# isislovecruft/aeonflux

Measured on AMD Instinct MI355X. Metric: credential presentations verified/sec, higher is better.
Workload: dtype int64

## Files before the change

aeonflux_amd/csrc/engine.cpp:

```cpp
#include "engine.hpp"
#include <stdio.h>
#include <string.h>
#include <algorithm>
#include <map>
#include <tuple>
#include <new>
#include <system_error>
#include <stdexcept>

namespace afx {

static thread_local std::string g_error;
void set_error(const std::string& s) { g_error = s; }
int exception_rc() noexcept {
  try {
    throw;
  } catch (const std::bad_alloc&) {
    try { set_error("out of host memory"); } catch (...) {}
    return AFX_E_NO_MEMORY;
  } catch (const std::system_error& e) {
    try { set_error(std::string("system: ") + e.what()); } catch (...) {}
    return AFX_E_NO_MEMORY;
  } catch (const std::exception& e) {
    try { set_error(std::string("internal: ") + e.what()); } catch (...) {}
// ... 18 lines not shown
    if (e != hipSuccess) { set_error(std::string("hipFree: ") + hipGetErrorString(e)); return AFX_E_HIP; }
  }
  const size_t want = (n + (size_t(1) << 20) - 1) & ~((size_t(1) << 20) - 1);
  hipError_t e = hipMalloc(&p, want);
  if (e != hipSuccess) { p = nullptr; g_alloc_failed = true; set_error("hipMalloc(" + std::to_string(want) + "): " + hipGetErrorString(e)); return AFX_E_HIP; }
  cap = want;
  return AFX_OK;
}
void DevBuf::release(bool wipe) {
  if (!p) return;
  if (wipe) (void)hipMemset(p, 0, cap);
  (void)hipFree(p);
  p = nullptr; cap = 0;
}

static void secure_zero(void* p, size_t n) {
  if (!n) return;
  memset(p, 0, n);
  __asm__ __volatile__("" : : "r"(p) : "memory");
}
Assembler::~Assembler() { secure_zero(blob_.data(), blob_.size()); }
static uint8_t* provisional_base(int range, int variant) { return (uint8_t*)(uintptr_t)(0x4000000000000000ull + ((uint64_t)(1 + range + 4 * variant) << 44)); }
Assembler::Assembler(afx_ctx* c, uint32_t cnt, int variant) : ctx(c), count(cnt) {
  blob_.reserve(1 << 16);
  blob_base_ = provisional_base(0, variant);
  ws_base_ = provisional_base(1, variant);
  blob_alloc(sizeof(afx_pass), 16);
  bad_ = (uint32_t*)ws_alloc(sizeof(uint32_t) * (size_t)count);
  Launch l;
  l.kind = L_FILL_BAD;
  l.njobs = 1;
  l.jobs_off = blob_alloc(sizeof(afx_fill_job), 16);
  launches.push_back(l);
}
uint8_t* Assembler::ws_alloc(size_t bytes) {
  const size_t off = (ws_off_ + 255) & ~size_t(255);
  ws_off_ = off + bytes;
  return ws_base_ + off;
}
int32_t* Assembler::new_var() { return (int32_t*)ws_alloc(sizeof(int32_t) * AFX_VAR_DWORDS * (size_t)count); }
uint8_t* Assembler::new_enc() { return ws_alloc(32 * (size_t)count); }
uint8_t* Assembler::new_wide() { return ws_alloc(64 * (size_t)count); }
uint8_t* Assembler::new_rows(size_t rows) { return ws_alloc(32 * rows * (size_t)count); }
uint64_t* Assembler::new_state() { return (uint64_t*)ws_alloc(sizeof(uint64_t) * 25 * (size_t)count); }
size_t Assembler::blob_alloc(size_t bytes, size_t align) {
  const size_t off = (blob_.size() + align - 1) & ~(align - 1);
  blob_.resize(off + bytes);
  return off;
}
template <class T> static void put_job(uint8_t* dst, const T& j) { memcpy(dst, &j, sizeof j); }
template <> void put_job(uint8_t* dst, const afx_decode_job& j) {
  afx_decode_job z; memset(&z, 0, sizeof z);
  z.enc = j.enc; z.out = j.out; z.reject_identity = j.reject_identity; z.elligator = j.elligator;
  memcpy(dst, &z, sizeof z);
}
template <> void put_job(uint8_t* dst, const afx_pointop_job& j) {
  afx_pointop_job z; memset(&z, 0, sizeof z);
  z.a = j.a; z.b = j.b; z.b_const = j.b_const; z.sa = j.sa; z.sb = j.sb; z.out = j.out; z.out_enc = j.out_enc; z.reject_identity = j.reject_identity;
  memcpy(dst, &z, sizeof z);
}
template <> void put_job(uint8_t* dst, const afx_scalarop_job& j) {
  afx_scalarop_job z; memset(&z, 0, sizeof z);
  z.a = j.a; z.a_stride = j.a_stride; z.b = j.b; z.b_stride = j.b_stride; z.c = j.c; z.c_stride = j.c_stride; z.negate = j.negate; z.out = j.out;
  memcpy(dst, &z, sizeof z);
}
template <LaunchKind K, class T>
void Assembler::add_jobs(const std::vector<T>& jobs) {
  static_assert(job_of_kind<T>(K), "not the job struct of this launch kind");
  if (jobs.empty()) return;
  Launch l;
  l.kind = K;
  l.njobs = (uint32_t)jobs.size();
  l.jobs_off = blob_alloc(sizeof(T) * jobs.size(), 16);
  for (size_t i = 0; i < jobs.size(); i++) put_job(blob_.data() + l.jobs_off + sizeof(T) * i, jobs[i]);
  launches.push_back(l);
}
void Assembler::decode(const std::vector<afx_decode_job>& jobs) {
  stats.decodings += jobs.size();
  stats.field_mul += AFX_DECODE_MUL * jobs.size();
  stats.field_sq += AFX_DECODE_SQ * jobs.size();
  stats.chain_mul += AFX_CHAIN_SQRT_MUL * jobs.size();
  stats.chain_sq += AFX_CHAIN_SQRT_SQ * jobs.size();
  if (!pending_maps_.empty()) {
    std::vector<afx_decode_job> all(pending_maps_);
    all.insert(all.end(), jobs.begin(), jobs.end());
    pending_maps_.clear();
    add_jobs(all);
    launches.back().odd = 1;
    flush_maps();
    return;
  }
  add_jobs(jobs);
}
void Assembler::flush_maps() {
  if (!pending_maps_.empty()) {
    std::vector<afx_decode_job> maps;
    maps.swap(pending_maps_);
    add_jobs(maps);
    launches.back().odd = 1;
  }
  if (!pending_map_sums_.empty()) {
    std::vector<afx_pointop_job> sums;
    sums.swap(pending_map_sums_);
    pointop(sums);
  }
}
void Assembler::sccheck(const std::vector<afx_sccheck_job>& jobs) { add_jobs(jobs); }
void Assembler::pointop(const std::vector<afx_pointop_job>& jobs) {
  flush_maps();
  for (const afx_pointop_job& j : jobs) {
    stats.var_additions += j.sb != 0;
    stats.encodings += j.out_enc != nullptr;
    stats.field_mul += (j.sb != 0 ? 9 : 0) + (j.out_enc ? AFX_ENCODE_MUL : 0);
    stats.field_sq += j.out_enc ? AFX_ENCODE_SQ : 0;
    stats.chain_mul += j.out_enc ? AFX_CHAIN_SQRT_MUL : 0;
    stats.chain_sq += j.out_enc ? AFX_CHAIN_SQRT_SQ : 0;
  }
  if (small() && (uint64_t)ctx->row_waves(count) * jobs.size() <= 2ull * 4 * ctx->n_cu) {
    std::vector<afx_pointop_job> moved(jobs);
    for (afx_pointop_job& j : moved) {
      if (!j.out_enc || j.reject_identity == 2) continue;
      if (!j.out) j.out = new_var();
      afx_compress_job cj = { j.out, j.out_enc, j.reject_identity, AFX_COMPRESS_PLAIN };
      pending_cjobs_.push_back(cj);
      j.out_enc = nullptr; j.reject_identity = 0;
    }
    add_jobs(moved);
    return;
  }
  add_jobs(jobs);
}
void Assembler::negenc(const std::vector<afx_negenc_job>& jobs) {
  flush_maps();
  if (jobs.empty()) return;
  stats.encodings += jobs.size();
  stats.field_mul += 11 + (2 * 3 + 2 + 17) * jobs.size();
  stats.field_sq += 254 + 3 * jobs.size();
  stats.chain_mul += AFX_CHAIN_INVERT_MUL; stats.chain_sq += AFX_CHAIN_INVERT_SQ;
  add_jobs(jobs);
  add_walk_rows(launches.back(), 0);
}
void Assembler::add_walk_rows(Launch& l, uint32_t per_row) {
  if (per_row == 0 || per_row > l.njobs) per_row = l.njobs;
  std::vector<afx_walk_row> rows;
  for (uint32_t first = 0; first < l.njobs; first += per_row) {
// ... 1329 lines not shown
```

aeonflux_amd/csrc/kernels.hip:

```cpp
#include <hip/hip_runtime.h>
#include "ge.cuh"
#include "keccak.cuh"
#include "plan.h"
#include "sc.cuh"
#include "sha512.cuh"

AFX_DEV void enc_load(uint32_t w[8], const uint8_t* arr, uint32_t item) {
  const uint4* p = reinterpret_cast<const uint4*>(arr + 32ull * item);
  const uint4 a = p[0], b = p[1];
  w[0] = a.x; w[1] = a.y; w[2] = a.z; w[3] = a.w; w[4] = b.x; w[5] = b.y; w[6] = b.z; w[7] = b.w;
}
AFX_DEV void enc_store(uint8_t* arr, uint32_t item, const uint32_t w[8]) {
  uint4* p = reinterpret_cast<uint4*>(arr + 32ull * item);
  p[0] = make_uint4(w[0], w[1], w[2], w[3]);
  p[1] = make_uint4(w[4], w[5], w[6], w[7]);
}
AFX_DEV sc sc_load_item(const uint8_t* arr, uint32_t stride, uint32_t item) {
  uint32_t w[8];
  enc_load(w, arr, stride ? item : 0);
  sc r;
#pragma unroll
  for (int i = 0; i < 8; i++) r.v[i] = w[i];
  return r;
}
// ... 115 lines not shown
    Q = ge_double(Q);
    if ((c >> bit) & 1u) Q = ge_p1p1_to_p3(ge_add_cached(Q, cB, false));
  }
#pragma unroll 1
  for (int k = 0; k < 4; k++) Q = ge_double(Q);
  int32_t* tab = postab + (size_t)(gj / windows) * windows * window_dwords + (size_t)(gj % windows) * window_dwords;
  const uint32_t first = c * AFX_POS_CHUNK, n = min((uint32_t)AFX_POS_CHUNK, entries - first);
  fe X[AFX_POS_CHUNK], Y[AFX_POS_CHUNK], Z[AFX_POS_CHUNK], pre[AFX_POS_CHUNK];
  fe prod = fe_one();
#pragma unroll 1
  for (uint32_t k = 0; k < n; k++) {
    X[k] = Q.X; Y[k] = Q.Y; Z[k] = Q.Z; pre[k] = prod;
    prod = fe_mul(prod, Q.Z);
    if (k + 1 < n) Q = ge_p1p1_to_p3(ge_add_cached(Q, cB, false));
  }
  fe inv = fe_invert(prod);
#pragma unroll 1
  for (int k = (int)n - 1; k >= 0; k--) {
    const fe zinv = fe_mul(inv, pre[k]);
    inv = fe_mul(inv, Z[k]);
    const ge_niels q = ge_niels_from_affine(fe_mul(X[k], zinv), fe_mul(Y[k], zinv));
    int32_t* e = tab + (size_t)(first + k) * AFX_NIELS_DWORDS;
#pragma unroll
    for (int l = 0; l < AFX_FE_LIMBS; l++) { e[l] = q.ypx.v[l]; e[9 + l] = q.ymx.v[l]; e[18 + l] = q.xyd.v[l]; }
    e[27] = 0;
  }
}

template <class T>
AFX_DEV const T* row_job(const T* __restrict__ jobs, const afx_row* __restrict__ rows) {
  if (rows) return reinterpret_cast<const T*>(reinterpret_cast<const uint8_t*>(jobs) + rows[blockIdx.y].job_off);
  return jobs + blockIdx.y;
}
AFX_DEV uint32_t row_pass_index(const afx_row* __restrict__ rows) { return rows ? rows[blockIdx.y].pass : 0u; }
template <class T> struct lane_row { T job; uint32_t count; uint32_t* bad; uint32_t item; };
template <class T>
AFX_DEV lane_row<T> lane_row_of(const T* __restrict__ jobs, const afx_row* __restrict__ rows, const afx_pass* __restrict__ passes) {
  const afx_pass pass = passes[row_pass_index(rows)];
  return { *row_job(jobs, rows), pass.count, pass.bad, blockIdx.x * blockDim.x + threadIdx.x };
}
AFX_DEV bool wave_past_end(uint32_t count) {
  return blockIdx.x * blockDim.x + ((uint32_t)__builtin_amdgcn_readfirstlane((int)threadIdx.x) & ~63u) >= count;
}
AFX_DEV uint32_t shadowing_item(uint32_t count) { return min(blockIdx.x * blockDim.x + threadIdx.x, count - 1); }
struct quad_seat { uint32_t lane, role, item; };
AFX_DEV quad_seat quad_seat_of(uint32_t count) {
  const uint32_t lane = threadIdx.x & 63u;
  return { lane, (uint32_t)__builtin_amdgcn_readfirstlane((int)(threadIdx.x >> 6)), min(blockIdx.x * 64u + lane, count - 1) };
}

AFX_DEV void decode_item(const afx_decode_job& job, uint32_t* bad, uint32_t count, uint32_t item) {
  uint32_t w[8];
  enc_load(w, job.enc, item);
  ge_p3 P;
  const bool ok = ristretto_decode(P, w);
  uint32_t flags = ok ? 0u : AFX_BAD_DECODE;
  if (job.reject_identity && is_identity_encoding(w)) flags |= AFX_BAD_IDENTITY;
  if (flags) atomicOr(&bad[item], flags);
  if (job.out) var_store(job.out, count, item, ok ? P : ge_identity());
}
__global__ void __launch_bounds__(AFX_BLOCK, 2) k_decode(const afx_decode_job* __restrict__ jobs, const afx_row* __restrict__ rows, const afx_pass* __restrict__ passes) {
  const auto [job, count, bad, item] = lane_row_of(jobs, rows, passes);
  if (item >= count) return;
  decode_item(job, bad, count, item);
}

__global__ void __launch_bounds__(AFX_BLOCK) k_decode_mixed(const afx_decode_job* __restrict__ jobs, const afx_row* __restrict__ rows, const afx_pass* __restrict__ passes) {
  const auto [job, count, bad, item] = lane_row_of(jobs, rows, passes);
  if (item >= count) return;
  if (job.elligator) {
    uint32_t w[8];
    enc_load(w, job.enc, 2 * item + (job.elligator - 1));
    var_store(job.out, count, item, ristretto_elligator(fe_frombytes(w)));
    return;
  }
  decode_item(job, bad, count, item);
}

__global__ void __launch_bounds__(AFX_BLOCK) k_sccheck(const afx_sccheck_job* __restrict__ jobs, const afx_row* __restrict__ rows, const afx_pass* __restrict__ passes) {
  const auto [job, count, bad, item] = lane_row_of(jobs, rows, passes);
  if (item >= count) return;
  const sc s = sc_load_item(job.sc, 32, item);
  if (!sc_is_canonical(s)) atomicOr(&bad[item], AFX_BAD_SCALAR);
}

__global__ void __launch_bounds__(AFX_BLOCK, 2) k_pointop(const afx_pointop_job* __restrict__ jobs, const afx_row* __restrict__ rows, const afx_pass* __restrict__ passes) {
  const auto [job, count, bad, item] = lane_row_of(jobs, rows, passes);
  if (item >= count) return;
  ge_p3 A = var_load(job.a, count, item);
  if (job.sa < 0) A = ge_neg(A);
  ge_p3 R = A;
  if (job.sb != 0) {
    const ge_p3 B = job.b ? var_load(job.b, count, item) : p3_load_uniform(job.b_const);
    R = ge_addsub(A, B, job.sb < 0);
  } else {
    R = ge_carry(R);
  }
  if (job.out) var_store(job.out, count, item, R);
  if (job.out_enc) {
    uint32_t w[8];
    ristretto_encode(w, R);
    enc_store(job.out_enc, item, w);
    if (job.reject_identity == 1 ? is_identity_encoding(w) : (job.reject_identity == 2 && !is_identity_encoding(w))) atomicOr(&bad[item], AFX_BAD_IDENTITY);
  }
}

// ... 1471 lines not shown
```

aeonflux_amd/csrc/launch_kinds.hpp:

```cpp
#pragma once
#include <stddef.h>
#include <stdint.h>
#include <string>
#include "../../include/aeonflux_gpu.h"
#include "kernels.h"
#include "plan.h"

hipError_t afxk_coef(hipStream_t s, const afx_coef_job* jobs, uint32_t njobs, const afx_row* rows, const afx_pass* passes, uint32_t max_count) __attribute__((weak));
hipError_t afxk_mask_rows(hipStream_t s, const afx_mask_job* jobs, uint32_t njobs, const afx_row* rows, const afx_pass* passes, uint32_t max_count) __attribute__((weak));
hipError_t afxk_sha512_jobs(hipStream_t s, const afx_sha512_job* jobs, uint32_t njobs, const afx_row* rows, const afx_pass* passes, uint32_t max_count) __attribute__((weak));
hipError_t afxk_encode_to_group(hipStream_t s, const afx_encode_job* jobs, uint32_t njobs, const afx_row* rows, const afx_pass* passes, uint32_t max_count) __attribute__((weak));
hipError_t afxk_encode_at(hipStream_t s, const afx_encode_at_job* jobs, uint32_t njobs, const afx_row* rows, const afx_pass* passes, uint32_t max_count) __attribute__((weak));
hipError_t afxk_sha512(hipStream_t s, const uint8_t* src, uint32_t stride, uint32_t offset, uint32_t len, uint8_t* out, uint32_t count) __attribute__((weak));
hipError_t afxk_draw(hipStream_t s, const afx_draw_job* jobs, uint32_t njobs, uint32_t max_count) __attribute__((weak));
hipError_t afxk_batch_weights(hipStream_t s, const uint8_t* seed, uint64_t index0, uint32_t label, uint32_t n_weights, uint32_t count, uint8_t* weights) __attribute__((weak));
hipError_t afxk_msg_gather(hipStream_t s, const afx_gather_job* job) __attribute__((weak));
hipError_t afxk_msg_expand(hipStream_t s, const afx_expand_job* job) __attribute__((weak));
hipError_t afxk_msg_status(hipStream_t s, const afx_msgstat_job* job) __attribute__((weak));
hipError_t afxk_sc_invert(hipStream_t s, const uint8_t* a, const uint8_t* b, uint8_t* out, uint32_t count) __attribute__((weak));
hipError_t afxk_tag_broadcast(hipStream_t s, const uint8_t* enc, uint8_t* rows, uint32_t count) __attribute__((weak));
hipError_t afxk_tag_scope_check(hipStream_t s, const uint8_t* enc, uint8_t* ok) __attribute__((weak));
hipError_t afxk_tagset_spend(hipStream_t s, const afx_tagset_table* t, const uint8_t* T, const uint8_t* status_in, uint32_t count, uint32_t* slot_of, uint8_t* seen_out)
    __attribute__((weak));
hipError_t afxk_tagset_contains(hipStream_t s, const afx_tagset_table* t, const uint8_t* T, uint32_t count, uint8_t* seen_out) __attribute__((weak));
// ... 19 lines not shown
  void fix(const T*& p) const { T* q = const_cast<T*>(p); fix(q); p = q; }
  template <class T, size_t N>
  void fix(T (&a)[N]) const { for (T& p : a) fix(p); }
};
template <class J, auto... M>
void fix_jobs(const Mover& m, uint8_t* j0, uint32_t n) {
  for (uint32_t i = 0; i < n; i++) {
    J& j = ((J*)j0)[i];
    (m.fix(j.*M), ...);
  }
}
enum OddRule { ODD_IGNORED, ODD_EQUAL, ODD_OR };

struct KindInfo {
  LaunchKind kind;
  const char* name;
  size_t job_size;
  const char* job_type;
  void (*fix)(const Mover& m, uint8_t* jobs, uint32_t njobs);
  bool walks;
  OddRule odd;
  int (*run)(const KindInfo& k, hipStream_t s, const uint8_t* jobs, uint32_t njobs, const afx_row* rows, const afx_pass* passes, uint32_t max_count);
  const char* call;
};

template <class J> constexpr const char* job_tag() { return __PRETTY_FUNCTION__; }
constexpr bool same_text(const char* a, const char* b) { while (*a && *a == *b) a++, b++; return *a == *b; }
template <class J>
using Launcher = hipError_t(hipStream_t, const J*, uint32_t, const afx_row*, const afx_pass*, uint32_t);
template <class J, Launcher<J>* F, bool OPTIONAL>
int run_common(const KindInfo& k, hipStream_t s, const uint8_t* jobs, uint32_t njobs, const afx_row* rows, const afx_pass* passes, uint32_t max_count) {
  if constexpr (OPTIONAL)
    if (!F) { set_error(std::string("no ") + k.name + " launcher in this build"); return AFX_E_NO_DEVICE; }
  const hipError_t e = F(s, (const J*)jobs, njobs, rows, passes, max_count);
  if (e != hipSuccess) { set_error(std::string(k.call) + ": " + hipGetErrorString(e)); return AFX_E_HIP; }
  return AFX_OK;
}
#define AFX_COMMON(J, F) &run_common<J, F, false>, #F "(s, (const " #J "*)jobs, nrows, rw, passes, max_count)"
#define AFX_OPTIONAL(J, F) &run_common<J, F, true>, #F "(s, (const " #J "*)jobs, nrows, rw, passes, max_count)"

template <class J, auto... M>
constexpr KindInfo kind_of(LaunchKind k, const char* name, bool walks = false, OddRule odd = ODD_IGNORED, decltype(KindInfo::run) run = nullptr, const char* call = nullptr) {
  return { k, name, sizeof(J), job_tag<J>(), &fix_jobs<J, M...>, walks, odd, run, call };
}
template <class J, auto... M>
constexpr KindInfo kind_of(LaunchKind k, const char* name, decltype(KindInfo::run) run, const char* call) { return kind_of<J, M...>(k, name, false, ODD_IGNORED, run, call); }

constexpr KindInfo msm_kind(LaunchKind k, const char* name) {
  return kind_of<afx_msm_djob, &afx_msm_djob::naf_sched, &afx_msm_djob::addend, &afx_msm_djob::out_enc, &afx_msm_djob::out_var, &afx_msm_djob::half_var>(k, name);
}

inline constexpr KindInfo KINDS[] = {
  kind_of<afx_fill_job, &afx_fill_job::p>(L_FILL_BAD, "k_fill_u32"),
  kind_of<afx_decode_job, &afx_decode_job::enc, &afx_decode_job::out>(L_DECODE, "k_decode", false, ODD_OR),
  kind_of<afx_sccheck_job, &afx_sccheck_job::sc>(L_SCCHECK, "k_sccheck", AFX_COMMON(afx_sccheck_job, afxk_sccheck)),
  kind_of<afx_pointop_job, &afx_pointop_job::a, &afx_pointop_job::b, &afx_pointop_job::b_const, &afx_pointop_job::out, &afx_pointop_job::out_enc>(
      L_POINTOP, "k_pointop", AFX_COMMON(afx_pointop_job, afxk_pointop)),
  kind_of<afx_scalarop_job, &afx_scalarop_job::a, &afx_scalarop_job::b, &afx_scalarop_job::c, &afx_scalarop_job::out>(
      L_SCALAROP, "k_scalarop", AFX_COMMON(afx_scalarop_job, afxk_scalarop)),
  msm_kind(L_MSM_WINDOW, "k_msm_window"),
  kind_of<afx_hash_program, &afx_hash_program::init_state, &afx_hash_program::load_state, &afx_hash_program::save_state, &afx_hash_program::records,
          &afx_hash_program::fields, &afx_hash_program::outs, &afx_hash_program::challenge, &afx_hash_program::trace>(L_HASH, "k_hash"),
  kind_of<afx_uniform_job, &afx_uniform_job::wide, &afx_uniform_job::out_enc, &afx_uniform_job::out_var>(
      L_FROM_UNIFORM, "k_from_uniform", AFX_COMMON(afx_uniform_job, afxk_from_uniform_jobs)),
  kind_of<afx_reduce_job, &afx_reduce_job::wide, &afx_reduce_job::out>(L_REDUCE_WIDE, "k_reduce_wide", AFX_COMMON(afx_reduce_job, afxk_reduce_wide_jobs)),
  { L_COPY, "copy", 0, nullptr, nullptr, false, ODD_IGNORED, nullptr, nullptr },
  kind_of<afx_finish_job, &afx_finish_job::bad, &afx_finish_job::status>(L_FINISH, "k_finish"),
  msm_kind(L_MSM_FIXED, "k_msm_fixed"),
  msm_kind(L_MSM_NAF, "k_msm_naf"),
  kind_of<afx_table_job, &afx_table_job::var>(L_MSM_TABLES, "k_msm_tables", false, ODD_EQUAL),
  kind_of<afx_compress_job, &afx_compress_job::var, &afx_compress_job::out_enc>(L_COMPRESS, "k_compress2x", true),
  kind_of<afx_pointsum_job, &afx_pointsum_job::parts, &afx_pointsum_job::addend, &afx_pointsum_job::out_var, &afx_pointsum_job::half_var, &afx_pointsum_job::out_enc>(
      L_POINTSUM, "k_pointsum", false, ODD_OR),
  kind_of<afx_negenc_job, &afx_negenc_job::enc, &afx_negenc_job::var, &afx_negenc_job::out_enc>(L_NEGENC, "k_negenc", true),
  kind_of<afx_table_job, &afx_table_job::var>(L_TABLE_AFFINE, "k_table_affine", true),
  kind_of<afx_powers_job, &afx_powers_job::src, &afx_powers_job::out>(L_POWERS, "k_powers", AFX_COMMON(afx_powers_job, afxk_powers)),
  kind_of<afx_coef_job, &afx_coef_job::weights, &afx_coef_job::triples, &afx_coef_job::operands, &afx_coef_job::out>(L_COEF, "k_coef", AFX_OPTIONAL(afx_coef_job, afxk_coef)),
  kind_of<afx_sha512_job, &afx_sha512_job::src, &afx_sha512_job::out, &afx_sha512_job::copy>(L_SHA512, "k_sha512", AFX_OPTIONAL(afx_sha512_job, afxk_sha512_jobs)),
  kind_of<afx_encode_job, &afx_encode_job::msgs, &afx_encode_job::M1, &afx_encode_job::counters, &afx_encode_job::zero_a, &afx_encode_job::zero_b>(
      L_ENCODE, "k_encode_to_group", AFX_OPTIONAL(afx_encode_job, afxk_encode_to_group)),
  kind_of<afx_mask_job, &afx_mask_job::p>(L_MASK, "k_mask_rows", AFX_OPTIONAL(afx_mask_job, afxk_mask_rows)),
  kind_of<afx_encode_at_job, &afx_encode_at_job::msgs, &afx_encode_at_job::counters_in, &afx_encode_at_job::M1, &afx_encode_at_job::zero_a, &afx_encode_at_job::zero_b>(
      L_ENCODE_AT, "k_encode_at", AFX_OPTIONAL(afx_encode_at_job, afxk_encode_at)),
};
#undef AFX_COMMON
#undef AFX_OPTIONAL
inline constexpr const char* TIMING_SLOT_NAMES[] = { "k_hash_coop", "k_hash_coop64", "k_sc_invert" };

constexpr bool kinds_in_enum_order() {
  for (int k = 0; k < (int)L_KINDS; k++) if (KINDS[k].kind != k) return false;
  return true;
}
static_assert(sizeof KINDS / sizeof KINDS[0] == L_KINDS && kinds_in_enum_order(), "one KINDS entry per launch kind, in the enum's order");
static_assert(sizeof TIMING_SLOT_NAMES / sizeof TIMING_SLOT_NAMES[0] == T_SLOTS - L_KINDS, "one name per timing slot past the launch kinds");
inline const KindInfo& kind_info(LaunchKind k) { return KINDS[k]; }
inline const char* timing_name(int slot) { return slot < (int)L_KINDS ? KINDS[slot].name : TIMING_SLOT_NAMES[slot - L_KINDS]; }

template <class J>
constexpr bool job_of_kind(LaunchKind k) { return KINDS[k].job_type && same_text(KINDS[k].job_type, job_tag<J>()); }
template <class J>
constexpr LaunchKind kind_of_job() {
  int found = L_KINDS, n = 0;
  for (int k = 0; k < (int)L_KINDS; k++) if (job_of_kind<J>((LaunchKind)k)) { found = k; n++; }
  return n == 1 ? (LaunchKind)found : L_KINDS;
}

}
// ... 1 lines not shown
```

aeonflux_amd/csrc/plan.h:

```cpp
#pragma once
#include <stdint.h>

#define AFX_KV_ONE_WAVE_CHAINS 0x08u
#define AFX_KV_HASH_HALF_WAVE 0x10u
#define AFX_KV_NO_POINTSUM_TREE 0x20u

#define AFX_CLOCK_SLOTS 64
#define AFX_MSM_MAX_TERMS 72
#define AFX_TABLE_ENTRIES 9
#define AFX_TABLE_STORED 8
#ifndef AFX_POS_BITS
#define AFX_POS_BITS 13
#endif
#define AFX_POS_WINDOWS ((253 + AFX_POS_BITS - 1) / AFX_POS_BITS)
#define AFX_POS_ENTRIES ((1 << (AFX_POS_BITS - 1)) + 1)
#define AFX_POS_WINDOW_DWORDS ((AFX_POS_ENTRIES * AFX_NIELS_DWORDS + 3) & ~3)
#define AFX_POS_TABLE_DWORDS (AFX_POS_WINDOWS * AFX_POS_WINDOW_DWORDS)
#define AFX_SEC_BITS 6
#define AFX_SEC_WINDOWS ((253 + AFX_SEC_BITS - 1) / AFX_SEC_BITS)
#define AFX_SEC_ENTRIES ((1 << (AFX_SEC_BITS - 1)) + 1)
#define AFX_SEC_WINDOW_DWORDS (AFX_SEC_ENTRIES * AFX_NIELS_DWORDS)
#define AFX_SEC_TABLE_DWORDS (AFX_SEC_WINDOWS * AFX_SEC_WINDOW_DWORDS)
#ifndef AFX_SECVAR_BITS
#define AFX_SECVAR_BITS 2
// ... 37 lines not shown
  uint32_t pass;
  uint32_t job_off;
} afx_row;

typedef struct {
  uint32_t job_off;
  uint32_t n_jobs;
  uint32_t pass, pad;
  int32_t* prefix_ws;
} afx_walk_row;

typedef struct { uint32_t* p; uint32_t v, n; } afx_fill_job;
typedef struct { const uint32_t* bad; uint8_t* status; uint32_t count, fail_code; } afx_finish_job;
typedef struct { uint8_t* p; } afx_mask_job;
typedef struct { const uint8_t* wide; uint8_t* out_enc; int32_t* out_var; } afx_uniform_job;
typedef struct { const uint8_t* wide; uint8_t* out; } afx_reduce_job;
typedef struct { const uint8_t* src; uint8_t* out; uint8_t* copy; uint32_t stride, offset, len, pad; } afx_sha512_job;
typedef struct { const uint8_t* msgs; uint8_t* M1; uint32_t* counters; uint8_t* zero_a; uint8_t* zero_b; } afx_encode_job;
typedef struct { const uint8_t* msgs; const uint32_t* counters_in; uint8_t* M1; uint8_t* zero_a; uint8_t* zero_b; } afx_encode_at_job;

typedef struct { const uint8_t* blob; const uint64_t* offsets; const uint32_t* chunk_first; uint8_t* rows; uint64_t bias; uint32_t count, n_chunks; } afx_gather_job;
#define AFX_EXPAND_MAX 3
typedef struct { const uint8_t* src[AFX_EXPAND_MAX]; uint8_t* dst[AFX_EXPAND_MAX]; const uint32_t* chunk_first; uint32_t count, n_chunks, n_rows; } afx_expand_job;
typedef struct {
  const uint8_t* chunk_status[2]; uint8_t* status; const uint32_t* chunk_first;
  const uint8_t* keys[AFX_EXPAND_MAX];
  uint8_t* rows32[2]; uint8_t* rows30; uint32_t* words;
  uint32_t count, n_chunks, n_keys, fail_code, phase, pad;
} afx_msgstat_job;

typedef struct { const uint8_t* seed; uint8_t* dst; uint64_t index; uint32_t count, label; } afx_draw_job;
#define AFX_DRAW_LEN(label) (((label) == 0u || (label) == 1u || (label) == 3u || ((label) >= 65u && (label) <= 67u) || (label) == 69u || \
                              ((label) >= 71u && (label) <= 102u)) ? 64u : 32u)

#define AFX_COEF_ONE 0xffffu
typedef struct { uint16_t weight, operand, negate, pad; } afx_coef_triple;
typedef struct {
  const uint8_t* weights;
  const afx_coef_triple* triples;
  const uint8_t* const* operands;
  uint8_t* out;
  uint64_t stride;
  uint32_t n_triples, pad;
} afx_coef_job;
#define AFX_WEIGHT_BYTES 16u

typedef int32_t* afx_var_t;

typedef struct {
  const uint8_t* enc;
  afx_var_t out;
  uint32_t reject_identity;
  uint32_t elligator;
} afx_decode_job;

typedef struct {
  const uint8_t* sc;
} afx_sccheck_job;

typedef struct {
  const int32_t* a;
  const int32_t* b;
  const int32_t* b_const;
  int32_t sa, sb;
  afx_var_t out;
  uint8_t* out_enc;
  uint32_t reject_identity;
} afx_pointop_job;

typedef struct {
  const uint8_t* a; uint32_t a_stride;
  const uint8_t* b; uint32_t b_stride;
  const uint8_t* c; uint32_t c_stride;
  uint32_t negate;
  uint8_t* out;
} afx_scalarop_job;

typedef struct {
  const uint8_t* scalar;
  uint32_t scalar_stride;
  int32_t fixed_idx;
  const int32_t* var;
  uint32_t negate;
  uint32_t table_slot;
  uint32_t secret;
  uint32_t dbl;
  uint32_t win_off;
  uint32_t pad;
} afx_msm_term;

typedef struct {
  uint32_t n_terms;
  uint32_t n_var;
  uint32_t n_uni;
  int32_t top_bit;
  const uint32_t* naf_sched;
  afx_msm_term term[AFX_MSM_MAX_TERMS];
  const int32_t* addend;
  uint32_t addend_negate;
  uint8_t* out_enc;
  afx_var_t out_var;
  uint32_t reject_identity;
  uint32_t leave_half;
  int32_t chain_to;
  afx_var_t half_var;
  uint32_t digit_slot;
// ... 119 lines not shown
```

aeonflux_amd/csrc/statements.cpp:

```cpp
#include <string.h>
#include <algorithm>
#include <functional>
#include <memory>
#include <stdexcept>
#include <vector>
#include "engine.hpp"
#include <stdlib.h>
#include "doors.hpp"

using namespace afx;

static const uint8_t SC_L_BYTES[32] = { 0xed, 0xd3, 0xf5, 0x5c, 0x1a, 0x63, 0x12, 0x58, 0xd6, 0x9c, 0xf7, 0xa2, 0xde, 0xf9, 0xde, 0x14,
                                        0, 0, 0, 0, 0, 0, 0, 0, 0, 0, 0, 0, 0, 0, 0, 0x10 };
static bool host_scalar_is_canonical(const uint8_t* s) {
  for (int i = 31; i >= 0; i--) {
    if (s[i] < SC_L_BYTES[i]) return true;
    if (s[i] > SC_L_BYTES[i]) return false;
  }
  return false;
}
static size_t sizeof_system_parameters(uint32_t n) { return n < 3 ? 32 * (5 + 3 + (size_t)n + 4) + 4 : 32 * (5 + 2 * (size_t)n + 4) + 4; }
static size_t sizeof_secret_key(uint32_t n) { return 32 * (5 + (size_t)n) + 4; }


// ... 330 lines not shown
      if (k >= 2) continue;
      if ((rc = L.blob_dev[i].ensure(BLOB_CAP))) return rc;
      AFX_HIP(hipHostMalloc(&L.blob_host[i], BLOB_CAP, hipHostMallocDefault));
      L.blob_host_cap[i] = BLOB_CAP;
    }
  for (auto& L : c->lane) AFX_HIP(hipEventCreateWithFlags(&L.msm_done, hipEventDisableTiming));
  std::vector<uint8_t> flat(32 * (size_t)c->ngen);
  for (uint32_t i = 0; i < c->ngen; i++) memcpy(flat.data() + 32 * (size_t)i, c->gen_enc[i].data(), 32);
  AFX_HIP(hipMemcpyAsync(c->d_gen_enc.p, flat.data(), flat.size(), hipMemcpyHostToDevice, c->stream));
  uint8_t* d_neg = (uint8_t*)c->lane[0].staging.p;
  uint32_t* d_ok = (uint32_t*)((uint8_t*)c->lane[0].staging.p + 32 * (size_t)c->ngen);
  AFX_HIP(afxk_setup_generators(c->stream, (const uint8_t*)c->d_gen_enc.p, c->ngen, (int32_t*)c->d_gen_ext.p, d_neg, d_ok));
  if ((rc = c->lane[0].ws.ensure(sizeof(int32_t) * AFX_VAR_DWORDS * (size_t)c->ngen * AFX_POS_WINDOWS))) return rc;
  AFX_HIP(afxk_setup_postables(c->stream, (const int32_t*)c->d_gen_ext.p, c->ngen, (int32_t*)c->lane[0].ws.p, (int32_t*)c->d_pos_tables.p, 0));
  std::vector<uint8_t> neg(32 * (size_t)c->ngen);
  std::vector<uint32_t> ok(c->ngen);
  AFX_HIP(hipMemcpyAsync(neg.data(), d_neg, neg.size(), hipMemcpyDeviceToHost, c->stream));
  AFX_HIP(hipMemcpyAsync(ok.data(), d_ok, 4 * (size_t)c->ngen, hipMemcpyDeviceToHost, c->stream));
  if (c->has_key) {
    std::vector<uint8_t> kflat(32 * (size_t)(4 + n));
    for (uint32_t i = 0; i < 4 + n; i++) memcpy(kflat.data() + 32 * (size_t)i, c->host_key[i].data(), 32);
    AFX_HIP(hipMemcpyAsync(c->d_key.p, kflat.data(), kflat.size(), hipMemcpyHostToDevice, c->stream));
    AFX_HIP(hipStreamSynchronize(c->stream));
    volatile uint8_t* p = kflat.data();
    for (size_t i = 0; i < kflat.size(); i++) p[i] = 0;
  }
  uint8_t consts[2048];
  memset(consts, 0, sizeof consts);
  consts[0] = 1;
  AFX_HIP(hipMemcpyAsync(c->d_consts.p, consts, sizeof consts, hipMemcpyHostToDevice, c->stream));
  AFX_HIP(hipStreamSynchronize(c->stream));
  for (uint32_t i = 0; i < c->ngen; i++)
    if (!ok[i]) { set_error("generator / key point " + std::to_string(i) + " does not decompress"); return AFX_E_BAD_PARAMS; }
  c->gen_neg_enc.assign(c->ngen, Enc{});
  for (uint32_t i = 0; i < c->ngen; i++) memcpy(c->gen_neg_enc[i].data(), neg.data() + 32 * (size_t)i, 32);
  if ((rc = build_secret_tables(c.get()))) return rc;
  *out = c.release();
  return AFX_OK;
}

extern "C" int afx_ctx_create(afx_ctx** out, int device, const uint8_t* sysparams, size_t sysparams_len, const uint8_t* amacs_key,
                              size_t amacs_key_len, const uint8_t issuer_params[64]) try {
  if (!issuer_params) { set_error("issuer_params is required"); return AFX_E_BAD_ARGS; }
  return afx_ctx_create_impl(out, device, sysparams, sysparams_len, amacs_key, amacs_key_len, nullptr, issuer_params);
} catch (...) { return afx::exception_rc(); }

struct BatchableIn {
  const uint8_t* main = nullptr;
  const uint8_t* const* enc = nullptr;
  uint32_t n_main = 0;
  const uint8_t* weights = nullptr;
  BatchableSum sum;
};
static void add_encproof_verify(Assembler& as, JobSets& js, uint16_t index, const afx_encproof_soa& e, size_t total, size_t off, uint32_t trace_row,
                                BatchableSum* sum = nullptr, const uint8_t* commitments = nullptr) {
  afx_ctx* c = as.ctx;
  auto row = [&](const uint8_t* base, size_t k) { return base + (k * total + off) * 32; };
  if (index >= c->n) { as.fail_all = true; return; }
  if (!sum) js.sccheck.push_back({ row(e.challenge, 0) });
  for (int k = 0; k < 6; k++) js.sccheck.push_back({ row(e.responses, k) });
  int32_t *v_pk = as.new_var(), *v_E1 = as.new_var(), *v_E2 = as.new_var(), *v_Cy1 = as.new_var(), *v_Cy2 = as.new_var(),
          *v_Cy3 = as.new_var(), *v_Cy2p = as.new_var(), *v_D1 = as.new_var();
  uint8_t *e_D1 = as.new_enc(), *e_D2 = as.new_enc();
  js.decode.push_back({ row(e.pk, 0), v_pk, 1 });
  js.decode.push_back({ row(e.E1, 0), v_E1, 1 });
  js.decode.push_back({ row(e.E2, 0), v_E2, 0 });
  js.decode.push_back({ row(e.C_y_1, 0), v_Cy1, 0 });
  js.decode.push_back({ row(e.C_y_2, 0), v_Cy2, 1 });
  js.decode.push_back({ row(e.C_y_3, 0), v_Cy3, 1 });
  js.decode.push_back({ row(e.C_y_2p, 0), v_Cy2p, 1 });
  afx_pointop_job d1 = { v_Cy1, v_E2, nullptr, +1, -1, v_D1, e_D1, 1 };
  js.pointop.push_back(d1);
  if (as.small()) js.pointop.push_back({ v_E1, nullptr, nullptr, -1, 0, nullptr, e_D2, 1 });
  else js.negenc.push_back({ row(e.E1, 0), v_E1, e_D2, 1, 0 });
  auto resp = [&](int k) { ScalarVar s; s.dev = row(e.responses, k); s.stride = 32; return s; };
  SchnorrBuilder v(as, "2019/1416 anonymous credentials", "2019/1416 proof of encryption");
  const int a = v.allocate_scalar("a", resp(0));
  const int a0 = v.allocate_scalar("a0", resp(1));
  const int a1 = v.allocate_scalar("a1", resp(2));
  const int m3 = v.allocate_scalar("m3", resp(3));
  const int z = v.allocate_scalar("z", resp(4));
  const int z1 = v.allocate_scalar("z1", resp(5));
  const int pk = v.allocate_point("pk", PointVar::Var(v_pk, row(e.pk, 0)));
  const int G_a = v.allocate_point("G_a", PointVar::Const(c->id_Ga()));
  const int G_a_0 = v.allocate_point("G_a_0", PointVar::Const(c->id_Ga0()));
  const int G_a_1 = v.allocate_point("G_a_1", PointVar::Const(c->id_Ga1()));
  const int G_y_1 = v.allocate_point("G_y_1", PointVar::Const(c->id_Gy(0)));
  const int G_y_2 = v.allocate_point("G_y_2", PointVar::Const(c->id_Gy(1)));
  const int G_y_3 = v.allocate_point("G_y_3", PointVar::Const(c->id_Gy(2)));
  const int G_m_3 = v.allocate_point("G_m_3", PointVar::Const(c->id_Gm(index)));
  const int C_y_2 = v.allocate_point("C_y_2", PointVar::Var(v_Cy2, row(e.C_y_2, 0)));
  const int C_y_3 = v.allocate_point("C_y_3", PointVar::Var(v_Cy3, row(e.C_y_3, 0)));
  const int C_y_2p = v.allocate_point("C_y_2'", PointVar::Var(v_Cy2p, row(e.C_y_2p, 0)));
  const int C_y_1_minus_E2 = v.allocate_point("C_y_1-E2", PointVar::Var(v_D1, e_D1));
  const int E1 = v.allocate_point("E1", PointVar::Var(v_E1, row(e.E1, 0)));
  const int minus_E1 = v.allocate_point("-E1", PointVar::NegOf(v_E1, e_D2));
  v.constrain(pk, { { a, G_a }, { a0, G_a_0 }, { a1, G_a_1 } });
  v.constrain(C_y_1_minus_E2, { { z, G_y_1 }, { a, minus_E1 } });
  v.constrain(C_y_2p, { { a1, C_y_2 } });
  v.constrain(E1, { { a0, C_y_2 }, { m3, C_y_2p }, { z1, G_y_2 } });
  v.constrain(C_y_3, { { z, G_y_3 }, { m3, G_m_3 } });
  if (sum) {
    const uint8_t* R[5];
    for (size_t j = 0; j < 5; j++) R[j] = row(commitments, j);
    if (!v.verify_batchable(R, 5, trace_row, total, off, *sum, js.decode, js.hash)) throw std::logic_error("a proof of encryption has five constraints");
    return;
  }
  v.verify_compact(row(e.challenge, 0), trace_row, total, off, js.msm1, js.hash);
}

static void add_tagproof_verify(Assembler& as, JobSets& js, std::vector<afx_msm_job>& chains, const TagVerify& tv, const int32_t* v_Cyp, size_t total, size_t off,
                                uint32_t trace_row) {
  afx_ctx* c = as.ctx;
  const uint32_t p = tv.position;
  if (p >= c->n) { as.fail_all = true; return; }
  auto row = [&](const uint8_t* base, size_t k) { return base + (k * total + off) * 32; };
  js.sccheck.push_back({ row(tv.nonce, 0) });
  js.sccheck.push_back({ row(tv.challenge, 0) });
  for (int k = 0; k < 2; k++) js.sccheck.push_back({ row(tv.responses, k) });
  int32_t *v_T = as.new_var(), *v_H = as.new_var(), *v_Cp = as.new_var();
// ... 35 lines not shown
    if (sh.kinds[i] > AFX_ENC_SECRET_POINT) return true;
  for (uint32_t j = 0; j < hs; j++)
    if (sh.hidden_scalar_indices[j] >= c->n) return true;
  for (uint32_t e = 0; e < sh.n_enc_proofs; e++)
    if (sh.enc_indices[e] >= c->n) return true;
  uint32_t k = 0;
  for (uint32_t i = 0; i < n; i++)
    if (sh.kinds[i] != AFX_ENC_SECRET_POINT) keep[k++] = i;
  if (c->strict) {
    uint32_t e = 0;
    for (uint32_t i = 0; i < n; i++)
      if (sh.kinds[i] == AFX_ENC_SECRET_POINT) {
        if (e >= sh.n_enc_proofs || sh.enc_indices[e] != i) return true;
        e++;
      }
    if (e != sh.n_enc_proofs) return true;
  }
  for (uint32_t j = 0; j < k; j++) {
    const uint32_t p = c->strict ? keep[j] : j;
    pos[j] = p;
    hidden_slot[j] = -1;
    if (sh.kinds[p] == AFX_ENC_SECRET_POINT) continue;
    if (p >= c->g) return true;
    if (sh.kinds[p] == AFX_ENC_SECRET_SCALAR) {
      for (uint32_t h = 0; h < hs; h++)
        if (sh.hidden_scalar_indices[h] == p) { hidden_slot[j] = (int)h; break; }
      if (hidden_slot[j] < 0) return true;
    }
  }
  *k_out = k;
  return false;
}

static void build_presentation_verify(Assembler& as, const afx_shape& sh, const afx_presentation_soa& b, size_t total, size_t off,
                                      uint8_t* status_dev, BatchableIn* bi = nullptr, const TagVerify* tv = nullptr) {
  afx_ctx* c = as.ctx;
  JobSets js;
  auto row = [&](const uint8_t* base, size_t k) { return base + (k * total + off) * 32; };
  const uint32_t n = sh.n_attributes, hs = sh.n_hidden_scalars;
  uint32_t keep[AFX_MAX_ATTRIBUTES], pos[AFX_MAX_ATTRIBUTES], k = 0;
  int hidden_slot[AFX_MAX_ATTRIBUTES];
  if (presentation_shape_rejects(c, sh, keep, &k, hidden_slot, pos)) as.fail_all = true;
  if (tv && (bi || !tagged_shape_ok(c, sh, tv->position))) as.fail_all = true;
  if (as.fail_all) { emit(as, js, status_dev, AFX_ST_VERIFICATION_FAILURE); return; }

  if (!bi) js.sccheck.push_back({ row(b.challenge, 0) });
  for (uint32_t r = 0; r < sh.n_responses; r++) js.sccheck.push_back({ row(b.responses, r) });
  int32_t *v_Cx0 = as.new_var(), *v_Cx1 = as.new_var(), *v_CV = as.new_var(), *v_A = as.new_var(), *v_Z = as.new_var();
  uint8_t* e_Z = as.new_enc();
  js.decode.push_back({ row(b.C_x_0, 0), v_Cx0, 1 });
  js.decode.push_back({ row(b.C_x_1, 0), v_Cx1, 1 });
  js.decode.push_back({ row(b.C_V, 0), v_CV, 0 });
  int32_t* v_Cy[AFX_MAX_ATTRIBUTES];
  std::vector<afx_msm_term> zterms;
  zterms.push_back(mk_term(c->key_x0(), 0, v_Cx0, -1, true));
  zterms.push_back(mk_term(c->key_x1(), 0, v_Cx1, -1, true));
  for (uint32_t i = 0; i < n; i++) {
    v_Cy[i] = as.new_var();
    js.decode.push_back({ row(b.C_y, i), v_Cy[i], sh.kinds[i] != AFX_ENC_SECRET_POINT ? 1u : 0u });
    const int32_t* X = v_Cy[i];
    if (sh.kinds[i] == AFX_ENC_PUBLIC_SCALAR) {
      js.sccheck.push_back({ row(b.attr_values, i) });
      uint8_t* ym = as.new_enc();
      afx_scalarop_job so;
      memset(&so, 0, sizeof so);
      so.a = c->key_y(i); so.a_stride = 0; so.b = row(b.attr_values, i); so.b_stride = 32; so.out = ym;
      js.scalarop.push_back(so);
      zterms.push_back(mk_term(ym, 32, nullptr, (int32_t)c->id_Gm(i), true));
    } else if (sh.kinds[i] == AFX_ENC_PUBLIC_POINT) {
      int32_t *v_M = as.new_var(), *v_X = as.new_var();
      js.decode.push_back({ row(b.attr_values, i), v_M, 0 });
      afx_pointop_job po = { v_Cy[i], v_M, nullptr, +1, +1, v_X, nullptr, 0 };
      js.pointop.push_back(po);
      X = v_X;
    }
    zterms.push_back(mk_term(c->key_y(i), 0, X, -1, true));
  }
  afx_pointop_job pa = { v_CV, nullptr, c->gen_ext(c->id_W()), +1, -1, v_A, nullptr, 0 };
  js.pointop.push_back(pa);
  afx_msm_job zj;
  memset(&zj, 0, sizeof zj);
  set_terms(zj, zterms);
  zj.addend = v_A;
  zj.out_var = v_Z;
  zj.out_enc = e_Z;
  zj.reject_identity = 1;
  const size_t z_index = js.msm1.size();
  js.msm1.push_back(zj);

  auto resp = [&](uint32_t r) { ScalarVar s; s.dev = row(b.responses, r); s.stride = 32; return s; };
  SchnorrBuilder v(as, "2019/1416 anonymous credential", "2019/1416 presentation proof");
  const int z = v.allocate_scalar("z", resp(0));
  const int z_0 = v.allocate_scalar("z_0", resp(1));
  const int t = v.allocate_scalar("t", resp(2));
  int H_s[AFX_MAX_ATTRIBUTES];
  for (uint32_t j = 0; j < hs; j++) H_s[j] = v.allocate_scalar("m", resp(3 + j));
  const int I = v.allocate_point("I", PointVar::Const(c->id_I()));
  const int C_x_1 = v.allocate_point("C_x_1", PointVar::Var(v_Cx1, row(b.C_x_1, 0)));
  const int C_x_0 = v.allocate_point("C_x_0", PointVar::Var(v_Cx0, row(b.C_x_0, 0)));
  const int G_x_0 = v.allocate_point("G_x_0", PointVar::Const(c->id_Gx0()));
  const int G_x_1 = v.allocate_point("G_x_1", PointVar::Const(c->id_Gx1()));
  int C_y[AFX_MAX_ATTRIBUTES], G_y[AFX_MAX_ATTRIBUTES], G_m[AFX_MAX_ATTRIBUTES];
  for (uint32_t j = 0; j < k; j++) C_y[j] = v.allocate_point("C_y", PointVar::Var(v_Cy[keep[j]], row(b.C_y, keep[j])));
  for (uint32_t i = 0; i < c->g; i++) G_y[i] = v.allocate_point("G_y", PointVar::Const(c->id_Gy(i)));
  for (uint32_t j = 0; j < hs; j++) G_m[j] = v.allocate_point("G_m", PointVar::Const(c->id_Gm(sh.hidden_scalar_indices[j])));
  int D[AFX_MAX_ATTRIBUTES], D_pos[AFX_MAX_ATTRIBUTES], nD = 0, neg_G_y_1 = -1;
  if (c->strict)
    for (uint32_t e = 0; e < sh.n_enc_proofs; e++) {
      const uint32_t i = sh.enc_indices[e];
      int32_t *v_C1 = as.new_var(), *v_D = as.new_var();
      uint8_t* e_D = as.new_enc();
      js.decode.push_back({ row(b.enc[e].C_y_1, 0), v_C1, 0 });
      afx_pointop_job dj = { v_Cy[i], v_C1, nullptr, +1, -1, v_D, e_D, i == 0 ? 2u  : 1u };
      js.pointop.push_back(dj);
      if (i == 0) continue;
      if (neg_G_y_1 < 0) neg_G_y_1 = v.allocate_point("-G_y_1", PointVar::Const(c->id_Gy(0), true));
      D[nD] = v.allocate_point("C_y-C_y_1", PointVar::Var(v_D, e_D));
      D_pos[nD++] = (int)i;
    }
  PointVar pZ = PointVar::Var(v_Z, e_Z);
  const bool expand_Z = !bi && as.small() && !c->secure_plan(false);
  if (expand_Z) {
    pZ.parts.push_back({ nullptr, 0, false, v_A, -1 });
    for (const afx_msm_term& t : zterms) pZ.parts.push_back({ t.scalar, t.scalar_stride, true, t.var, t.fixed_idx });
  }
  const int Z = v.allocate_point("Z", pZ);
  v.constrain(Z, { { z, I } });
  v.constrain(C_x_1, { { t, C_x_0 }, { z_0, G_x_0 }, { z, G_x_1 } });
  for (uint32_t j = 0; j < k; j++) {
    const uint32_t p = pos[j];
    if (sh.kinds[p] == AFX_ENC_SECRET_POINT) continue;
    if (sh.kinds[p] == AFX_ENC_SECRET_SCALAR) v.constrain(C_y[j], { { z, G_y[p] }, { H_s[hidden_slot[j]], G_m[hidden_slot[j]] } });
    else v.constrain(C_y[j], { { z, G_y[p] } });
  }
  for (int d = 0; d < nD; d++) v.constrain(D[d], { { z, G_y[D_pos[d]] }, { z, neg_G_y_1 } });
  if (bi) {
    std::vector<const uint8_t*> R(v.num_constraints());
    for (size_t j = 0; j < R.size(); j++) R[j] = row(bi->main, j);
    if (!v.verify_batchable(R.data(), bi->n_main, 0, total, off, bi->sum, js.decode, js.hash)) {
      as.plan_error = "the shape's main proof does not have that many commitments";
      as.finish(status_dev, AFX_ST_VERIFICATION_FAILURE);
      return;
    }
    for (uint32_t e = 0; e < sh.n_enc_proofs; e++) add_encproof_verify(as, js, sh.enc_indices[e], b.enc[e], total, off, 1 + e, &bi->sum, bi->enc[e]);
    as.sccheck(js.sccheck);
    as.decode(js.decode);
    as.scalarop(js.scalarop);
    as.pointop(js.pointop);
    as.negenc(js.negenc);
    as.msm(js.msm1);
    as.hash(js.hash);
    std::vector<afx_coef_job> coefs;
    std::vector<afx_msm_job> sums;
    std::vector<int32_t*> parts = bi->sum.emit(as, bi->weights + off * AFX_WEIGHT_BYTES, total, coefs, sums);
    as.coef(coefs);
    as.msm(sums);
    const int32_t* acc = parts.at(0);
    for (size_t k = 1; k + 1 < parts.size(); k++) {
      int32_t* nv = as.new_var();
      const afx_pointop_job add = { acc, parts[k], nullptr, +1, +1, nv, nullptr, 0 };
      as.pointop({ add });
      acc = nv;
    }
    const afx_pointop_job last = { acc, parts.size() > 1 ? parts.back() : nullptr, nullptr, +1, parts.size() > 1 ? +1 : 0, nullptr, as.new_enc(), 2u };
    as.pointop({ last });
    as.finish(status_dev, AFX_ST_VERIFICATION_FAILURE);
    return;
  }
  const size_t first_constraint = js.msm1.size();
  v.verify_compact(row(b.challenge, 0), 0, total, off, js.msm1, js.hash, nullptr, expand_Z ? &js.scalarop2 : nullptr);
  if (!expand_Z) js.msm1[z_index].chain_to = (int32_t)first_constraint;
  for (uint32_t e = 0; e < sh.n_enc_proofs && !as.fail_all; e++) add_encproof_verify(as, js, sh.enc_indices[e], b.enc[e], total, off, 1 + e);
  if (tv && !as.fail_all) add_tagproof_verify(as, js, js.msm2, *tv, v_Cy[tv->position], total, off, 1 + sh.n_enc_proofs);
  emit(as, js, status_dev, AFX_ST_VERIFICATION_FAILURE);
}

int verify_presentations_dev_impl(afx_ctx* ctx, const afx_shape* shape, const afx_presentation_soa* batch, size_t count, uint8_t* status_dev, const TagVerify* tag) {
  CtxLock lock__(ctx);
  if (!ctx || !shape || !batch || !status_dev) { set_error("null argument"); return AFX_E_BAD_ARGS; }
  if (!ctx->has_key) { set_error("Issuer::verify needs the issuer key"); return AFX_E_NO_KEY; }
  if (count == 0) return AFX_OK;
  if (shape->n_enc_proofs && shape->n_enc_proofs <= AFX_MAX_ATTRIBUTES && !batch->enc) { set_error("enc proofs missing"); return AFX_E_BAD_ARGS; }
  const afx_shape sh = *shape;
  const afx_presentation_soa b = *batch;
  {
    uint32_t keep[AFX_MAX_ATTRIBUTES], pos[AFX_MAX_ATTRIBUTES], k = 0;
    int slot[AFX_MAX_ATTRIBUTES];
    if (!presentation_shape_rejects(ctx, sh, keep, &k, slot, pos)) {
      bool missing = !b.challenge || !b.C_x_0 || !b.C_x_1 || !b.C_V || (sh.n_attributes && !b.C_y) || (sh.n_responses && !b.responses);
      for (uint32_t i = 0; i < sh.n_attributes; i++)
        if ((sh.kinds[i] == AFX_ENC_PUBLIC_SCALAR || sh.kinds[i] == AFX_ENC_PUBLIC_POINT) && !b.attr_values) missing = true;
      for (uint32_t e = 0; e < sh.n_enc_proofs; e++) {
        const afx_encproof_soa& q = b.enc[e];
        missing |= !q.challenge || !q.responses || !q.pk || !q.E1 || !q.E2 || !q.C_y_1 || !q.C_y_2 || !q.C_y_3 || !q.C_y_2p;
      }
      if (tag && tagged_shape_ok(ctx, sh, tag->position)) missing |= !tag->H_rows || !tag->nonce || !tag->T || !tag->challenge || !tag->responses;
      if (missing) { set_error("null batch array"); return AFX_E_BAD_ARGS; }
    }
  }
  std::vector<afx_encproof_soa> encs;
  if (b.enc && sh.n_enc_proofs <= AFX_MAX_ATTRIBUTES) encs.assign(b.enc, b.enc + sh.n_enc_proofs);
  const afx_shape csh = canonical_shape(sh);
  struct { afx_shape sh; uint32_t p; } kt;
  memset(&kt, 0, sizeof kt);
  kt.sh = csh; kt.p = tag ? tag->position : 0;
  const PlanKey key = ctx->trace ? PlanKey() : tag ? plan_key("verify_presentations_tagged", &kt, sizeof kt, mode_flags(ctx))
                                                   : plan_key("verify_presentations", &csh, sizeof csh, mode_flags(ctx));
  return run_chunked(ctx, count, [&](Assembler& as, size_t off, uint32_t) {
    afx_presentation_soa bb = b;
    bb.enc = encs.data();
    build_presentation_verify(as, sh, bb, count, off, status_dev + off, nullptr, tag);
  }, key);
}
extern "C" int afx_verify_presentations_dev(afx_ctx* ctx, const afx_shape* shape, const afx_presentation_soa* batch, size_t count,
                                            uint8_t* status_dev) try {
  return verify_presentations_dev_impl(ctx, shape, batch, count, status_dev, nullptr);
} catch (...) { return afx::exception_rc(); }

int verify_tag_proofs_dev_impl(afx_ctx* ctx, const TagVerify& tag, const uint8_t* C_y_p, size_t count, uint8_t* status_dev) {
  CtxLock lock__(ctx);
  if (!ctx || !status_dev) { set_error("null argument"); return AFX_E_BAD_ARGS; }
  if (count == 0) return AFX_OK;
  if (tag.position < ctx->n && (!C_y_p || !tag.H_rows || !tag.nonce || !tag.T || !tag.challenge || !tag.responses)) { set_error("null batch array"); return AFX_E_BAD_ARGS; }
  const uint32_t kp = tag.position;
  const PlanKey key = ctx->trace ? PlanKey() : plan_key("verify_tag_proofs", &kp, sizeof kp, mode_flags(ctx));
// ... 371 lines not shown
```

Before: 2.857 million.

## Skip redundant ristretto decodes when a row's encoding matches an earlier decoded row

```diff
diff --git a/aeonflux_amd/csrc/engine.cpp b/aeonflux_amd/csrc/engine.cpp
--- a/aeonflux_amd/csrc/engine.cpp
+++ b/aeonflux_amd/csrc/engine.cpp
@@ -94,6 +94,7 @@
 template <> void put_job(uint8_t* dst, const afx_decode_job& j) {
   afx_decode_job z; memset(&z, 0, sizeof z);
   z.enc = j.enc; z.out = j.out; z.reject_identity = j.reject_identity; z.elligator = j.elligator;
+  z.same_as_enc = j.same_as_enc; z.same_as_var = j.same_as_var;
   memcpy(dst, &z, sizeof z);
 }
 template <> void put_job(uint8_t* dst, const afx_pointop_job& j) {
@@ -123,16 +124,28 @@
   stats.field_sq += AFX_DECODE_SQ * jobs.size();
   stats.chain_mul += AFX_CHAIN_SQRT_MUL * jobs.size();
   stats.chain_sq += AFX_CHAIN_SQRT_SQ * jobs.size();
+  std::vector<afx_decode_job> first, copies;
+  for (afx_decode_job j : jobs) {
+    if (j.same_as_enc && j.same_as_var && !small()) { copies.push_back(j); continue; }
+    j.same_as_enc = nullptr; j.same_as_var = nullptr;
+    first.push_back(j);
+  }
+  for (const afx_decode_job& c : copies) {
+    bool found = false;
+    for (const afx_decode_job& o : first) found |= o.enc == c.same_as_enc && o.out == c.same_as_var && o.reject_identity == c.reject_identity && !o.elligator;
+    if (!found || c.elligator || !c.out) throw std::logic_error("a decode job repeats a row that its call does not decode with the same options");
+  }
   if (!pending_maps_.empty()) {
     std::vector<afx_decode_job> all(pending_maps_);
-    all.insert(all.end(), jobs.begin(), jobs.end());
+    all.insert(all.end(), first.begin(), first.end());
     pending_maps_.clear();
     add_jobs(all);
     launches.back().odd = 1;
     flush_maps();
-    return;
-  }
-  add_jobs(jobs);
+  } else {
+    add_jobs(first);
+  }
+  add_jobs(copies);
 }
 void Assembler::flush_maps() {
   if (!pending_maps_.empty()) {
diff --git a/aeonflux_amd/csrc/kernels.hip b/aeonflux_amd/csrc/kernels.hip
--- a/aeonflux_amd/csrc/kernels.hip
+++ b/aeonflux_amd/csrc/kernels.hip
@@ -191,6 +191,17 @@
 AFX_DEV void decode_item(const afx_decode_job& job, uint32_t* bad, uint32_t count, uint32_t item) {
   uint32_t w[8];
   enc_load(w, job.enc, item);
+  if (job.same_as_enc) {
+    uint32_t o[8];
+    enc_load(o, job.same_as_enc, item);
+    uint32_t diff = 0;
+#pragma unroll
+    for (int k = 0; k < 8; k++) diff |= w[k] ^ o[k];
+    if (diff == 0) {
+      var_store(job.out, count, item, var_load(job.same_as_var, count, item));
+      return;
+    }
+  }
   ge_p3 P;
   const bool ok = ristretto_decode(P, w);
   uint32_t flags = ok ? 0u : AFX_BAD_DECODE;
diff --git a/aeonflux_amd/csrc/launch_kinds.hpp b/aeonflux_amd/csrc/launch_kinds.hpp
--- a/aeonflux_amd/csrc/launch_kinds.hpp
+++ b/aeonflux_amd/csrc/launch_kinds.hpp
@@ -95,7 +95,7 @@
 
 inline constexpr KindInfo KINDS[] = {
   kind_of<afx_fill_job, &afx_fill_job::p>(L_FILL_BAD, "k_fill_u32"),
-  kind_of<afx_decode_job, &afx_decode_job::enc, &afx_decode_job::out>(L_DECODE, "k_decode", false, ODD_OR),
+  kind_of<afx_decode_job, &afx_decode_job::enc, &afx_decode_job::out, &afx_decode_job::same_as_enc, &afx_decode_job::same_as_var>(L_DECODE, "k_decode", false, ODD_OR),
   kind_of<afx_sccheck_job, &afx_sccheck_job::sc>(L_SCCHECK, "k_sccheck", AFX_COMMON(afx_sccheck_job, afxk_sccheck)),
   kind_of<afx_pointop_job, &afx_pointop_job::a, &afx_pointop_job::b, &afx_pointop_job::b_const, &afx_pointop_job::out, &afx_pointop_job::out_enc>(
       L_POINTOP, "k_pointop", AFX_COMMON(afx_pointop_job, afxk_pointop)),
diff --git a/aeonflux_amd/csrc/plan.h b/aeonflux_amd/csrc/plan.h
--- a/aeonflux_amd/csrc/plan.h
+++ b/aeonflux_amd/csrc/plan.h
@@ -113,6 +113,8 @@
   afx_var_t out;
   uint32_t reject_identity;
   uint32_t elligator;
+  const uint8_t* same_as_enc;
+  const int32_t* same_as_var;
 } afx_decode_job;
 
 typedef struct {
diff --git a/aeonflux_amd/csrc/statements.cpp b/aeonflux_amd/csrc/statements.cpp
--- a/aeonflux_amd/csrc/statements.cpp
+++ b/aeonflux_amd/csrc/statements.cpp
@@ -406,8 +406,13 @@
   const uint8_t* weights = nullptr;
   BatchableSum sum;
 };
+struct DecodedRow { const uint8_t* enc = nullptr; const int32_t* var = nullptr; uint32_t reject_identity = 0; };
+static afx_decode_job repeat_of(afx_decode_job j, const DecodedRow* orig) {
+  if (orig && orig->enc && orig->var && orig->reject_identity == j.reject_identity) { j.same_as_enc = orig->enc; j.same_as_var = orig->var; }
+  return j;
+}
 static void add_encproof_verify(Assembler& as, JobSets& js, uint16_t index, const afx_encproof_soa& e, size_t total, size_t off, uint32_t trace_row,
-                                BatchableSum* sum = nullptr, const uint8_t* commitments = nullptr) {
+                                BatchableSum* sum = nullptr, const uint8_t* commitments = nullptr, const DecodedRow* C_y = nullptr, DecodedRow* pk0 = nullptr) {
   afx_ctx* c = as.ctx;
   auto row = [&](const uint8_t* base, size_t k) { return base + (k * total + off) * 32; };
   if (index >= c->n) { as.fail_all = true; return; }
@@ -416,10 +421,11 @@
   int32_t *v_pk = as.new_var(), *v_E1 = as.new_var(), *v_E2 = as.new_var(), *v_Cy1 = as.new_var(), *v_Cy2 = as.new_var(),
           *v_Cy3 = as.new_var(), *v_Cy2p = as.new_var(), *v_D1 = as.new_var();
   uint8_t *e_D1 = as.new_enc(), *e_D2 = as.new_enc();
-  js.decode.push_back({ row(e.pk, 0), v_pk, 1 });
+  js.decode.push_back(repeat_of({ row(e.pk, 0), v_pk, 1 }, pk0));
+  if (pk0 && !pk0->enc) *pk0 = { row(e.pk, 0), v_pk, 1 };
   js.decode.push_back({ row(e.E1, 0), v_E1, 1 });
   js.decode.push_back({ row(e.E2, 0), v_E2, 0 });
-  js.decode.push_back({ row(e.C_y_1, 0), v_Cy1, 0 });
+  js.decode.push_back(repeat_of({ row(e.C_y_1, 0), v_Cy1, 0 }, C_y));
   js.decode.push_back({ row(e.C_y_2, 0), v_Cy2, 1 });
   js.decode.push_back({ row(e.C_y_3, 0), v_Cy3, 1 });
   js.decode.push_back({ row(e.C_y_2p, 0), v_Cy2p, 1 });
@@ -561,12 +567,14 @@
   js.decode.push_back({ row(b.C_x_1, 0), v_Cx1, 1 });
   js.decode.push_back({ row(b.C_V, 0), v_CV, 0 });
   int32_t* v_Cy[AFX_MAX_ATTRIBUTES];
+  DecodedRow d_Cy[AFX_MAX_ATTRIBUTES], d_pk0;
   std::vector<afx_msm_term> zterms;
   zterms.push_back(mk_term(c->key_x0(), 0, v_Cx0, -1, true));
   zterms.push_back(mk_term(c->key_x1(), 0, v_Cx1, -1, true));
   for (uint32_t i = 0; i < n; i++) {
     v_Cy[i] = as.new_var();
-    js.decode.push_back({ row(b.C_y, i), v_Cy[i], sh.kinds[i] != AFX_ENC_SECRET_POINT ? 1u : 0u });
+    d_Cy[i] = { row(b.C_y, i), v_Cy[i], sh.kinds[i] != AFX_ENC_SECRET_POINT ? 1u : 0u };
+    js.decode.push_back({ d_Cy[i].enc, v_Cy[i], d_Cy[i].reject_identity });
     const int32_t* X = v_Cy[i];
     if (sh.kinds[i] == AFX_ENC_PUBLIC_SCALAR) {
       js.sccheck.push_back({ row(b.attr_values, i) });
@@ -614,12 +622,13 @@
   for (uint32_t i = 0; i < c->g; i++) G_y[i] = v.allocate_point("G_y", PointVar::Const(c->id_Gy(i)));
   for (uint32_t j = 0; j < hs; j++) G_m[j] = v.allocate_point("G_m", PointVar::Const(c->id_Gm(sh.hidden_scalar_indices[j])));
   int D[AFX_MAX_ATTRIBUTES], D_pos[AFX_MAX_ATTRIBUTES], nD = 0, neg_G_y_1 = -1;
+  auto Cy_of = [&](uint32_t e) -> const DecodedRow* { return sh.enc_indices[e] == 0 && n > 0 ? &d_Cy[0] : nullptr; };
   if (c->strict)
     for (uint32_t e = 0; e < sh.n_enc_proofs; e++) {
       const uint32_t i = sh.enc_indices[e];
       int32_t *v_C1 = as.new_var(), *v_D = as.new_var();
       uint8_t* e_D = as.new_enc();
-      js.decode.push_back({ row(b.enc[e].C_y_1, 0), v_C1, 0 });
+      js.decode.push_back(repeat_of({ row(b.enc[e].C_y_1, 0), v_C1, 0 }, i == 0 ? &d_Cy[0] : nullptr));
       afx_pointop_job dj = { v_Cy[i], v_C1, nullptr, +1, -1, v_D, e_D, i == 0 ? 2u  : 1u };
       js.pointop.push_back(dj);
       if (i == 0) continue;
@@ -651,7 +660,7 @@
       as.finish(status_dev, AFX_ST_VERIFICATION_FAILURE);
       return;
     }
-    for (uint32_t e = 0; e < sh.n_enc_proofs; e++) add_encproof_verify(as, js, sh.enc_indices[e], b.enc[e], total, off, 1 + e, &bi->sum, bi->enc[e]);
+    for (uint32_t e = 0; e < sh.n_enc_proofs; e++) add_encproof_verify(as, js, sh.enc_indices[e], b.enc[e], total, off, 1 + e, &bi->sum, bi->enc[e], Cy_of(e), &d_pk0);
     as.sccheck(js.sccheck);
     as.decode(js.decode);
     as.scalarop(js.scalarop);
@@ -679,7 +688,7 @@
   const size_t first_constraint = js.msm1.size();
   v.verify_compact(row(b.challenge, 0), 0, total, off, js.msm1, js.hash, nullptr, expand_Z ? &js.scalarop2 : nullptr);
   if (!expand_Z) js.msm1[z_index].chain_to = (int32_t)first_constraint;
-  for (uint32_t e = 0; e < sh.n_enc_proofs && !as.fail_all; e++) add_encproof_verify(as, js, sh.enc_indices[e], b.enc[e], total, off, 1 + e);
+  for (uint32_t e = 0; e < sh.n_enc_proofs && !as.fail_all; e++) add_encproof_verify(as, js, sh.enc_indices[e], b.enc[e], total, off, 1 + e, nullptr, nullptr, Cy_of(e), &d_pk0);
   if (tv && !as.fail_all) add_tagproof_verify(as, js, js.msm2, *tv, v_Cy[tv->position], total, off, 1 + sh.n_enc_proofs);
   emit(as, js, status_dev, AFX_ST_VERIFICATION_FAILURE);
 }
```

Result: no change. 2.870 million, median of 6 (+0.5%).
